# vsois/hanabi-agents

Hardware: AMD Instinct MI355X
Metric: env_steps_per_sec (higher is better)
Workload: dtype u8 env/encoder + bfloat16 Q-net GEMM (fp32 accumulate, fp32 master weights)

## Files before the change

### hanabi-agents_amd/csrc/actor_fused.hip

```cpp
#include <hip/hip_runtime.h>
#include <hip/hip_bf16.h>
#include <hip/hip_fp16.h>

#include <cstdint>
#include <type_traits>

#include "../../include/hanabi_hip.h"
#include "common.hpp"
#include "env_kernel.hpp"

using hb::fail;

namespace {

typedef __bf16 bf16x8 __attribute__((ext_vector_type(8)));
typedef _Float16 f16x8 __attribute__((ext_vector_type(8)));
typedef float f32x4 __attribute__((ext_vector_type(4)));

constexpr int FM = 128;
constexpr int FH = 512;
constexpr int FNT = 512;
constexpr int FK = 51;
constexpr int S2 = FH / 32;
constexpr int LUT_BYTES = 65536;
constexpr int H_BYTES = FM * FH * 2;
constexpr int FRAG_FLOATS = 3 * 8 * FM;
constexpr int LDS_TOTAL = H_BYTES + FRAG_FLOATS * 4;
constexpr float NEG_BIG = -1e30f;

struct FusedArgs {
  const uint32_t* obs;
  long long m;
  int words;
  int s1;
  const uint4* w1f;
  const float* b1;
  const uint4* w2f;
  const float* b2;
  const float* support;
  float* q;
  int n_actions, n_pass;
  const int8_t* legal;
  int32_t* actions;
  float epsilon;
  unsigned long long seed, draw;
  long long first_gid;
  unsigned long long* stamps;
};

#if defined(__HIP_DEVICE_COMPILE__)
typedef const __attribute__((address_space(4))) unsigned char KargByte;
typedef const __attribute__((address_space(4))) hb::EnvArgs KargEnv;
constexpr size_t ENV_KARG_OFF = (sizeof(FusedArgs) + alignof(hb::EnvArgs) - 1) / alignof(hb::EnvArgs) * alignof(hb::EnvArgs);
#define HB_ENV_KARGS(NAME)                                            \
  auto NAME##_kargs_ = __builtin_amdgcn_kernarg_segment_ptr();        \
  asm volatile("" : "+s"(NAME##_kargs_));                             \
  KargEnv& NAME = *(KargEnv*)((KargByte*)NAME##_kargs_ + ENV_KARG_OFF)
#else
#define HB_ENV_KARGS(NAME) const hb::EnvArgs NAME{}
#endif

#ifdef HB_STAMPS
#define HB_FSTAMP(slot)                                                                              \
  do {                                                                                               \
    __builtin_amdgcn_sched_barrier(0);                                                               \
    unsigned long long hb_t_;                                                                        \
    asm volatile("s_memtime %0\n\ts_waitcnt lgkmcnt(0)" : "=s"(hb_t_)::"memory");                    \
    if (a.stamps && lane == 0) a.stamps[(static_cast<long long>(blockIdx.x) * 8 + wave) * 16 + (slot)] = hb_t_; \
    __builtin_amdgcn_sched_barrier(0);                                                               \
  } while (0)
#define HB_FSTAMP_REAL(slot)                                                                         \
  do {                                                                                               \
    unsigned long long hb_t_;                                                                        \
    asm volatile("s_memrealtime %0\n\ts_waitcnt lgkmcnt(0)" : "=s"(hb_t_)::"memory");                \
    if (a.stamps && lane == 0) a.stamps[(static_cast<long long>(blockIdx.x) * 8 + wave) * 16 + (slot)] = hb_t_; \
  } while (0)
#else
#define HB_FSTAMP(slot) do {} while (0)
#define HB_FSTAMP_REAL(slot) do {} while (0)
#endif

template <bool F16>
__device__ __forceinline__ uint32_t pack16(float lo, float hi) {
  if constexpr (F16) {
    const _Float16 a = static_cast<_Float16>(lo), b = static_cast<_Float16>(hi);
    uint16_t ua, ub;
    __builtin_memcpy(&ua, &a, 2);
    __builtin_memcpy(&ub, &b, 2);
    return static_cast<uint32_t>(ua) | (static_cast<uint32_t>(ub) << 16);
  } else {
    const __hip_bfloat16 a = __float2bfloat16(lo), b = __float2bfloat16(hi);
    return static_cast<uint32_t>(*reinterpret_cast<const uint16_t*>(&a)) |
           (static_cast<uint32_t>(*reinterpret_cast<const uint16_t*>(&b)) << 16);
  }
}
template <bool F16>
__device__ __forceinline__ uint32_t bits2_one(uint32_t b, int p) {
  const uint32_t t = (b >> (2 * p)) & 3u;
  return __umul24((t | (t << 15)) & 0x00010001u, F16 ? 0x3C00u : 0x3F80u);
}
template <bool F16>
__device__ __forceinline__ f32x4 mfma16(const uint4& wv, const uint4& xv, const f32x4& c) {
  if constexpr (F16) {
    union { uint4 u; f16x8 f; } w, x;
    w.u = wv; x.u = xv;
    return __builtin_amdgcn_mfma_f32_16x16x32_f16(w.f, x.f, c, 0, 0, 0);
  } else {
    union { uint4 u; bf16x8 f; } w, x;
    w.u = wv; x.u = xv;
    return __builtin_amdgcn_mfma_f32_16x16x32_bf16(w.f, x.f, c, 0, 0, 0);
  }
}
typedef float f32x2 __attribute__((ext_vector_type(2)));
typedef unsigned int u32x2 __attribute__((ext_vector_type(2)));
__device__ __forceinline__ float vmax(float a, float b) {
  float r;
  asm("v_max_f32 %0, %1, %2" : "=v"(r) : "v"(a), "v"(b));
  return r;
}
__device__ __forceinline__ float vmax3(float a, float b, float c) {
  float r;
  asm("v_max3_f32 %0, %1, %2, %3" : "=v"(r) : "v"(a), "v"(b), "v"(c));
  return r;
}
__device__ __forceinline__ float exp2_fast(float x) { return __builtin_amdgcn_exp2f(x); }

template <bool F16, class K, int EG>
__device__ __forceinline__ void actor_fused_body(const FusedArgs& a) {
  __shared__ __attribute__((aligned(16))) unsigned char lds[LDS_TOTAL];
  const int tid = threadIdx.x, lane = tid & 63;
  const int wave = __builtin_amdgcn_readfirstlane(tid >> 6);
  const int r = lane & 15, qd = lane >> 4;
  const long long row0 = static_cast<long long>(blockIdx.x) * FM;
  const int s1 = a.s1, G = (s1 + 3) >> 2;
  unsigned char* lutb = lds + (LDS_TOTAL - LUT_BYTES);
  const int bits_off = LDS_TOTAL - LUT_BYTES - 2048 * G;
  unsigned char* bits = lds + bits_off;
  const int m_early = bits_off >> 14;

  HB_FSTAMP_REAL(14);
  HB_FSTAMP(0);
  const uint4* w1p = a.w1f + (4 * wave) * 64 + lane;
  uint4 wa[4], wb[4];
#pragma unroll
  for (int n = 0; n < 4; ++n) wa[n] = w1p[n * 64];

  uint32_t w[4] = {0u, 0u, 0u, 0u};
  auto load_item = [&](int it) {
    const int rr = it & (FM - 1), g = it >> 7;
    long long row = row0 + rr;
    if (row >= a.m) row = a.m - 1;
    const uint32_t* src = a.obs + row * a.words + 4 * g;
#pragma unroll
    for (int i = 0; i < 4; ++i) w[i] = (4 * g + i < a.words) ? src[i] : 0u;
  };
  if (tid < FM * G) load_item(tid);
  for (int e = tid; e < 4096; e += FNT) {
    const uint32_t v = static_cast<uint32_t>(e) >> 4;
    *reinterpret_cast<uint4*>(lutb + e * 16) = make_uint4(bits2_one<F16>(v, 0), bits2_one<F16>(v, 1), bits2_one<F16>(v, 2), bits2_one<F16>(v, 3));
  }
  for (int it = tid; it < FM * G; it += FNT) {
    const int rr = it & (FM - 1), g = it >> 7;
    if (it != tid) load_item(it);
    uint32_t* dst = reinterpret_cast<uint32_t*>(bits) + (static_cast<size_t>((rr >> 4) * G + g) * 64 + (rr & 15));
#pragma unroll
    for (int qq = 0; qq < 4; ++qq) {
      const uint32_t o = ((w[0] >> (8 * qq)) & 0xFFu) | (((w[1] >> (8 * qq)) & 0xFFu) << 8) | (((w[2] >> (8 * qq)) & 0xFFu) << 16) |
                         (((w[3] >> (8 * qq)) & 0xFFu) << 24);
      dst[qq * 16] = o;
    }
  }
  HB_FSTAMP(1);
  __syncthreads();
  HB_FSTAMP(2);

  f32x4 acc[4][8];
#pragma unroll
  for (int n = 0; n < 4; ++n) {
    const float4 b = *reinterpret_cast<const float4*>(a.b1 + 64 * wave + 16 * n + 4 * qd);
#pragma unroll
    for (int m = 0; m < 8; ++m) acc[n][m] = f32x4{b.x, b.y, b.z, b.w};
  }

  {
    const unsigned char* lut = lutb + r * 16;
    const uint32_t* bw = reinterpret_cast<const uint32_t*>(bits) + lane;
#define HB_L1_STEP(I, WCUR, WNXT, HAVE_NEXT)                                                                   \
  {                                                                                                            \
    const int s_ = 4 * g + (I);                                                                                \
    if (HAVE_NEXT) {                                                                                           \
      _Pragma("unroll") for (int n = 0; n < 4; ++n) WNXT[n] = w1p[(s_ + 1) * 2048 + n * 64];                    \
    }                                                                                                          \
// ... 44 lines not shown
  HB_FSTAMP(4);
  __syncthreads();
  HB_H_WRITE(m >= m_early)
#undef HB_H_WRITE

  HB_FSTAMP(5);
  __syncthreads();
  HB_FSTAMP(6);

  const int n_pass = a.n_pass, A = a.n_actions;
  const int full_cap = 8 * n_pass;
  constexpr float LOG2E = 1.44269504088896340736f;
  const unsigned char* hrow = lds + r * 1024;

  for (int p = 0; p < n_pass; ++p) {
    const int slot = 8 * p + wave;
    {
      const float* bp = a.b2 + static_cast<long long>(slot) * 64 + 4 * qd;
#pragma unroll
      for (int n = 0; n < 4; ++n) {
        const float4 b = *reinterpret_cast<const float4*>(bp + 16 * n);
#pragma unroll
        for (int m = 0; m < 8; ++m) acc[n][m] = f32x4{b.x, b.y, b.z, b.w};
      }
    }
    const uint4* wp = w2p + static_cast<long long>(p) * S2 * 2048;
#define HB_L2_HALF(S, WCUR, M0)                                                                                \
  {                                                                                                            \
    uint4 xf[4];                                                                                               \
    const int ch = ((4 * (S) + qd) ^ r) << 4;                                                                  \
    _Pragma("unroll") for (int m = 0; m < 4; ++m) xf[m] = *reinterpret_cast<const uint4*>(hrow + ((M0) + m) * 16384 + ch); \
    _Pragma("unroll") for (int n = 0; n < 4; ++n) {                                                            \
      _Pragma("unroll") for (int m = 0; m < 4; ++m)                                                            \
        acc[n][(M0) + m] = mfma16<F16>(WCUR[n], xf[m], acc[n][(M0) + m]);                                      \
    }                                                                                                          \
  }
#define HB_L2_STEP(S, WCUR, WNXT, HAVE_NEXT)                                                                   \
  {                                                                                                            \
    if (HAVE_NEXT) {                                                                                           \
      _Pragma("unroll") for (int n = 0; n < 4; ++n) WNXT[n] = wp[((S) + 1) * 2048 + n * 64];                    \
    }                                                                                                          \
    asm volatile("" ::: "memory");                                                                             \
    HB_L2_HALF(S, WCUR, 0)                                                                                     \
    __builtin_amdgcn_sched_barrier(0);                                                                         \
    HB_L2_HALF(S, WCUR, 4)                                                                                     \
  }
#pragma unroll 1
    for (int s = 0; s < S2; s += 2) {
      HB_L2_STEP(s, wa, wb, true)
      HB_L2_STEP(s + 1, wb, wa, (s + 2 < S2))
    }
#undef HB_L2_STEP
#undef HB_L2_HALF
    if (p < 2) HB_FSTAMP(7 + 3 * p);
    if (p + 1 < n_pass) {
#pragma unroll
      for (int n = 0; n < 4; ++n) wa[n] = wp[S2 * 2048 + n * 64];
    }

    auto sup_at = [&](int k) { return a.support[k < FK ? k : FK - 1]; };
    f32x2 supF[6];
#pragma unroll
    for (int i = 0; i < 6; ++i) supF[i] = f32x2{sup_at(4 * (2 * i) + qd), sup_at(4 * (2 * i + 1) + qd)};
    const float supF12 = sup_at(48 + qd);
    const int fq = wave & 3;
    const f32x2 supZa = f32x2{sup_at(13 * fq + qd), sup_at(13 * fq + 4 + qd)};
    const f32x2 supZb = f32x2{sup_at(13 * fq + 8 + qd), sup_at(13 * fq + 12)};
    const bool full_ok = slot < A && slot < full_cap;
    float* fb = reinterpret_cast<float*>(lds + H_BYTES) + wave * FM;
    const f32x2 L2 = f32x2{LOG2E, LOG2E};
    hb::static_for<2>([&](auto MH) {
    constexpr int M0 = 4 * decltype(MH)::value;
    float qF[4], zm[4], zs[4], zt[4], vf12[4], vz3[4], nmx[4], nmz[4];
#define HB_M for (int m = 0; m < 4; ++m)
#define HB_SWAP16(X, OP) { const u32x2 t_ = __builtin_amdgcn_permlane16_swap(__float_as_uint(X), __float_as_uint(X), false, false); \
                           X = OP(__uint_as_float(t_.x), __uint_as_float(t_.y)); }
#define HB_SWAP32(X, OP) { const u32x2 t_ = __builtin_amdgcn_permlane32_swap(__float_as_uint(X), __float_as_uint(X), false, false); \
                           X = OP(__uint_as_float(t_.x), __uint_as_float(t_.y)); }
#define HB_ADD(A_, B_) ((A_) + (B_))
#pragma unroll
    HB_M { vf12[m] = qd < 3 ? acc[3][M0 + m][0] : NEG_BIG; vz3[m] = qd == 3 ? acc[3][M0 + m][0] : NEG_BIG; }
#pragma unroll
    HB_M nmx[m] = vmax3(acc[0][M0 + m][0], acc[0][M0 + m][1], acc[0][M0 + m][2]);
#pragma unroll
    HB_M nmx[m] = vmax3(nmx[m], acc[0][M0 + m][3], acc[1][M0 + m][0]);
#pragma unroll
    HB_M nmx[m] = vmax3(nmx[m], acc[1][M0 + m][1], acc[1][M0 + m][2]);
#pragma unroll
    HB_M nmx[m] = vmax3(nmx[m], acc[1][M0 + m][3], acc[2][M0 + m][0]);
#pragma unroll
    HB_M nmx[m] = vmax3(nmx[m], acc[2][M0 + m][1], acc[2][M0 + m][2]);
#pragma unroll
    HB_M nmx[m] = vmax3(nmx[m], acc[2][M0 + m][3], vf12[m]);
#pragma unroll
    HB_M nmz[m] = vmax(vmax3(acc[3][M0 + m][1], acc[3][M0 + m][2], acc[3][M0 + m][3]), vz3[m]);
#pragma unroll
    HB_M HB_SWAP16(nmx[m], vmax)
#pragma unroll
    HB_M HB_SWAP16(nmz[m], vmax)
#pragma unroll
    HB_M HB_SWAP32(nmx[m], vmax)
#pragma unroll
    HB_M HB_SWAP32(nmz[m], vmax)
#pragma unroll
    HB_M { nmx[m] *= -LOG2E; nmz[m] *= -LOG2E; }
    f32x2 s2[4], t2[4];
#define HB_PAIR_FIRST(N, LO, SUP)                                                                   \
// ... 25 lines not shown
      sF[m] = s2[m].x + s2[m].y + e12;
      tF[m] = t2[m].x + t2[m].y + e12 * supF12;
    }
#pragma unroll
    HB_M {
      const f32x2 arg = f32x2{acc[3][M0 + m][1], acc[3][M0 + m][2]} * L2 + f32x2{nmz[m], nmz[m]};
      const f32x2 e = f32x2{exp2_fast(arg.x), exp2_fast(arg.y)};
      s2[m] = e;
      t2[m] = e * supZa;
    }
#pragma unroll
    HB_M {
      const f32x2 arg = f32x2{acc[3][M0 + m][3], vz3[m]} * L2 + f32x2{nmz[m], nmz[m]};
      const f32x2 e = f32x2{exp2_fast(arg.x), exp2_fast(arg.y)};
      s2[m] += e;
      t2[m] += e * supZb;
    }
#pragma unroll
    HB_M { zs[m] = s2[m].x + s2[m].y; zt[m] = t2[m].x + t2[m].y; }
#pragma unroll
    HB_M HB_SWAP16(sF[m], HB_ADD)
#pragma unroll
    HB_M HB_SWAP16(tF[m], HB_ADD)
#pragma unroll
    HB_M HB_SWAP16(zs[m], HB_ADD)
#pragma unroll
    HB_M HB_SWAP16(zt[m], HB_ADD)
#pragma unroll
    HB_M HB_SWAP32(sF[m], HB_ADD)
#pragma unroll
    HB_M HB_SWAP32(tF[m], HB_ADD)
#pragma unroll
    HB_M HB_SWAP32(zs[m], HB_ADD)
#pragma unroll
    HB_M HB_SWAP32(zt[m], HB_ADD)
#pragma unroll
    HB_M { zm[m] = -nmz[m]; qF[m] = tF[m] * __builtin_amdgcn_rcpf(sF[m]) * (1.0f / FK); }
#undef HB_M
#undef HB_SWAP16
#undef HB_SWAP32
#undef HB_ADD
    if (qd == 0) {
#pragma unroll
      for (int m = 0; m < 4; ++m) {
        const long long row = row0 + 16 * (M0 + m) + r;
        if (full_ok && row < a.m) a.q[row * A + slot] = qF[m];
        fb[16 * (M0 + m) + r] = zm[m];
        fb[8 * FM + 16 * (M0 + m) + r] = zs[m];
        fb[16 * FM + 16 * (M0 + m) + r] = zt[m];
      }
    }
    __builtin_amdgcn_sched_barrier(0);
    });
    if (p < 2) HB_FSTAMP(8 + 3 * p);
    __syncthreads();
    if (tid < 2 * FM) {
      const int rr = tid & (FM - 1), g = tid >> 7;
      const int ea = full_cap + 2 * p + g;
      const long long row = row0 + rr;
      if (ea < A && row < a.m) {
        const float* f = reinterpret_cast<const float*>(lds + H_BYTES) + (4 * g) * FM + rr;
        const float m0 = f[0], m1 = f[FM], m2 = f[2 * FM], m3 = f[3 * FM];
        const float M = fmaxf(fmaxf(m0, m1), fmaxf(m2, m3));
        const float e0 = exp2_fast(m0 - M), e1 = exp2_fast(m1 - M), e2 = exp2_fast(m2 - M), e3 = exp2_fast(m3 - M);
        const float* fs = f + 8 * FM;
        const float* ft = f + 16 * FM;
        const float S = fs[0] * e0 + fs[FM] * e1 + fs[2 * FM] * e2 + fs[3 * FM] * e3;
        const float T = ft[0] * e0 + ft[FM] * e1 + ft[2 * FM] * e2 + ft[3 * FM] * e3;
        a.q[row * A + ea] = T * __builtin_amdgcn_rcpf(S) * (1.0f / FK);
      }
    }
    if (p + 1 < n_pass) __syncthreads();
    if (p < 2) HB_FSTAMP(9 + 3 * p);
  }
  [[maybe_unused]] uint32_t rf_flag[2] = {0u, 0u}, rf_ep[2] = {0u, 0u};
  if constexpr (!std::is_void_v<K>) {
    if (wave >= 2) {
      HB_ENV_KARGS(env);
#pragma unroll
      for (int h = 0; h < 2; ++h) {
        const long long g = row0 + 64 * h + lane;
        if (g < env.n) {
          rf_flag[h] = env.refill[g];
          rf_ep[h] = env.state[g * K::SW + 6];
        }
      }
    }
  }
  if (a.legal) {
    asm volatile("s_waitcnt vmcnt(0)" ::: "memory");
    __syncthreads();
    if (tid < FM && row0 + tid < a.m) {
      const long long g = row0 + tid;
      const unsigned long long gid = static_cast<unsigned long long>(a.first_gid + g);
      uint32_t rnd[4];
      hb::philox4x32_10(static_cast<uint32_t>(a.draw), static_cast<uint32_t>(a.draw >> 32), static_cast<uint32_t>(gid),
                        static_cast<uint32_t>(gid >> 32), static_cast<uint32_t>(a.seed), static_cast<uint32_t>(a.seed >> 32), rnd);
      const float* qr = a.q + g * A;
      const int8_t* lr = a.legal + g * A;
      float best = -INFINITY;
      unsigned long long legal_mask = 0, ties = 0;
      for (int i = 0; i < A; ++i) {
        const float v = __hip_atomic_load(qr + i, __ATOMIC_RELAXED, __HIP_MEMORY_SCOPE_AGENT);
        if (lr[i] != 0) {
          legal_mask |= 1ull << i;
          if (v > best) { best = v; ties = 1ull << i; }
          else if (v == best) ties |= 1ull << i;
        }
      }
      const float u = static_cast<float>(rnd[0] >> 8) * (1.0f / 16777216.0f);
      unsigned long long pool = (u < a.epsilon) ? legal_mask : ties;
      if (pool == 0) pool = legal_mask;
      int pick = 0;
      const int c = __popcll(pool);
      if (c > 0) {
        int k = static_cast<int>(__umulhi(rnd[1], static_cast<uint32_t>(c)));
        while (k-- > 0) pool &= pool - 1;
        pick = __ffsll(static_cast<long long>(pool)) - 1;
      }
      a.actions[g] = pick;
      if constexpr (!std::is_void_v<K>) reinterpret_cast<int*>(lds + H_BYTES)[tid] = pick;
    }
  }
  if constexpr (!std::is_void_v<K>) {
    static_assert(K::LIFE >= 2, "a deck flagged by one launch is regenerated by the next: a game must outlive the step after its deal");
    if (wave >= 2) {
      HB_ENV_KARGS(env);
      int turn = wave - 2;
#pragma unroll
      for (int h = 0; h < 2; ++h) {
        unsigned long long todo = __ballot(rf_flag[h] != 0u);
        while (todo) {
          const int src = __ffsll(static_cast<long long>(todo)) - 1;
          todo &= todo - 1;
          if (turn == 0) {
            const long long g = row0 + 64 * h + src;
            hb::refill_deck<K>(env, g, lane, [&] {
              return static_cast<uint32_t>(__builtin_amdgcn_readlane(static_cast<int>(rf_ep[h]), src));
            });
            if (lane == 0) env.refill[g] = 0;
            turn = 6;
          }
          --turn;
        }
      }
      asm volatile("s_waitcnt vmcnt(0)" ::: "memory");
    }
    constexpr int ENV_WORDS = hb::env_lds_words<K, EG>();
    static_assert((FM / EG) * ENV_WORDS * 4 <= H_BYTES && FM / EG <= FNT / 64, "env tail: the LDS slices must fit in H");
    __syncthreads();
    if (wave < FM / EG) {
      HB_ENV_KARGS(env);
      const long long g0 = row0 + EG * wave;
      const int uid = lane < EG ? reinterpret_cast<const int*>(lds + H_BYTES)[EG * wave + lane] : 0;
      hb::env_wave_step<K, EG>(env, g0, lane, reinterpret_cast<uint32_t*>(lds) + wave * ENV_WORDS, uid, g0 / EG);
    }
  }
  HB_FSTAMP_REAL(15);
}

template <bool F16>
__global__ __launch_bounds__(FNT) void actor_fused_kernel(const FusedArgs a) {
  actor_fused_body<F16, void, 16>(a);
}

template <bool F16, class K, int EG>
__global__ __launch_bounds__(FNT) void actor_env_fused_kernel(const FusedArgs a, const hb::EnvArgs env) {
  (void)env;
  actor_fused_body<F16, K, EG>(a);
}

template <bool F16>
__global__ __launch_bounds__(FNT) void actor_fused_grouped_kernel(const FusedArgs a, const hb_fused_tile* __restrict__ tiles) {
  const hb_fused_tile& t = tiles[blockIdx.x];
  if (!t.active) return;
  FusedArgs b = a;
  b.w1f = static_cast<const uint4*>(t.w1f); b.b1 = t.b1f; b.w2f = static_cast<const uint4*>(t.w2f); b.b2 = t.b2f;
  b.support = t.support;
  b.first_gid = t.first_game_id - static_cast<long long>(blockIdx.x) * FM;
  actor_fused_body<F16, void, 16>(b);
}

struct PackArgs {
  const __hip_bfloat16* w1; int w1_ld;
  const __hip_bfloat16* b1;
  const __hip_bfloat16* w2; int w2_ld;
  const __hip_bfloat16* b2;
  int obs_len, s1, n_actions, n_pass;
  uint4* w1f; float* b1f; uint4* w2f; float* b2f;
  int chunks1, chunks2;
  int f16;
  uint16_t* w1t; int w1t_ld;
  uint16_t* w2t; int w2t_ld;
};
__device__ __forceinline__ float bias_to_float(const __hip_bfloat16* b, int i, int f16) {
  return f16 ? __half2float(reinterpret_cast<const __half*>(b)[i]) : __bfloat162float(b[i]);
}
__host__ __device__ __forceinline__ int fused_logit(int col, int n_actions, int n_pass) {
  const int slot = col >> 6, c = col & 63, n = c >> 4, q = (c >> 2) & 3, j = c & 3;
  const int r16 = 4 * n + j;
  const int full_cap = 8 * n_pass;
  int action, atom;
  if (r16 < 12 || (r16 == 12 && q < 3)) {
    action = slot < full_cap ? slot : n_actions;
    if (action >= n_actions) return -1;
    atom = r16 < 12 ? 4 * r16 + q : 48 + q;
  } else {
    const int p = slot >> 3, w = slot & 7, f = w & 3;
    action = full_cap + 2 * p + (w >> 2);
    atom = r16 == 12 ? 13 * f + 12 : 13 * f + 4 * (r16 - 13) + q;
// ... 197 lines not shown
    a.first_gid = sel->first_gid;
  }
  *launch = true;
  return HB_OK;
}

static int fused_launch(const uint32_t* obs_bits_dev, int64_t n_rows, int32_t obs_len, const void* w1f_dev, const float* b1f_dev,
                        const void* w2f_dev, const float* b2f_dev, const float* support_dev, int32_t hidden, int32_t n_actions,
                        int32_t n_atoms, float* q_dev, unsigned long long* stamps_dev, const FusedSelect* sel, int32_t dtype, void* stream) {
  FusedArgs a;
  bool go = false;
  if (int rc = fused_args(obs_bits_dev, n_rows, obs_len, w1f_dev, b1f_dev, w2f_dev, b2f_dev, support_dev, hidden, n_actions, n_atoms, q_dev,
                          stamps_dev, sel, dtype, a, &go))
    return rc;
  if (!go) return HB_OK;
  const dim3 grid(static_cast<unsigned>((n_rows + FM - 1) / FM));
  if (dtype == 2) hipLaunchKernelGGL(actor_fused_kernel<true>, grid, dim3(FNT), 0, static_cast<hipStream_t>(stream), a);
  else hipLaunchKernelGGL(actor_fused_kernel<false>, grid, dim3(FNT), 0, static_cast<hipStream_t>(stream), a);
  HB_HIP(hipGetLastError());
  return HB_OK;
}

}

namespace {

using ActEnvFull2 = hb::Cfg<2, 5, 5, 5, 8, 3>;
using ActEnvFull5 = hb::Cfg<5, 5, 5, 4, 8, 3>;
constexpr int ENV_EG = 16;

template <class K>
static bool is_cfg(const hb::EnvVariant& v) {
  return v.P == K::P && v.C == K::C && v.R == K::R && v.H == K::H && v.INFO == K::INFO && v.LIFE == K::LIFE;
}

template <bool F16, class K>
static void launch_act_env(const FusedArgs& a, const hb::EnvArgs& env, dim3 grid, hipStream_t stream) {
  if (env.ev_start && env.ev_stop)
    hipExtLaunchKernelGGL((actor_env_fused_kernel<F16, K, ENV_EG>), grid, dim3(FNT), 0, stream, env.ev_start, env.ev_stop, 0, a, env);
  else
    hipLaunchKernelGGL((actor_env_fused_kernel<F16, K, ENV_EG>), grid, dim3(FNT), 0, stream, a, env);
}

}

namespace hb {

bool actor_env_fused_supported(const EnvVariant& v) { return is_cfg<ActEnvFull2>(v) || is_cfg<ActEnvFull5>(v); }

int actor_env_fused_launch(const uint32_t* obs_bits_dev, const int8_t* legal_dev, int64_t n_rows, int32_t obs_len, const void* w1f_dev,
                           const float* b1f_dev, const void* w2f_dev, const float* b2f_dev, const float* support_dev, int32_t hidden,
                           int32_t n_actions, int32_t n_atoms, float* q_dev, float epsilon, uint64_t seed, uint64_t draw,
                           int64_t first_game_id, int32_t* actions_dev, int32_t dtype, const EnvArgs& env, const EnvVariant& var,
                           void* stream) {
  if (!legal_dev || !actions_dev) return fail(HB_ERR_INVALID, "null argument");
  if (!actor_env_fused_supported(var)) return fail(HB_ERR_INVALID, "no fused policy + env kernel for this game configuration");
  if (n_rows != env.n) return fail(HB_ERR_INVALID, "n_rows (%lld) must equal the env's game count (%lld)", static_cast<long long>(n_rows), env.n);
  if (n_actions != var.n_actions || obs_len != var.obs_len) return fail(HB_ERR_INVALID, "actor shape does not match the env");
  const FusedSelect sel{legal_dev, actions_dev, epsilon, seed, draw, first_game_id};
  FusedArgs a;
  bool go = false;
  if (int rc = fused_args(obs_bits_dev, n_rows, obs_len, w1f_dev, b1f_dev, w2f_dev, b2f_dev, support_dev, hidden, n_actions, n_atoms, q_dev,
                          nullptr, &sel, dtype, a, &go))
    return rc;
  if (!go) return HB_OK;
  const dim3 grid(static_cast<unsigned>((n_rows + FM - 1) / FM));
  const hipStream_t st = static_cast<hipStream_t>(stream);
  const bool f16 = dtype == 2;
  if (is_cfg<ActEnvFull2>(var)) {
    if (f16) launch_act_env<true, ActEnvFull2>(a, env, grid, st);
    else launch_act_env<false, ActEnvFull2>(a, env, grid, st);
  } else {
    if (f16) launch_act_env<true, ActEnvFull5>(a, env, grid, st);
    else launch_act_env<false, ActEnvFull5>(a, env, grid, st);
  }
  HB_HIP(hipGetLastError());
  return HB_OK;
}

}
```

### hanabi-agents_amd/csrc/env_api.hip

```cpp
#include <hip/hip_runtime.h>

#include <cstdarg>
#include <cstdio>
#include <cstdlib>
#include <cstring>
#include <new>
#include <string>
#include <vector>

#include "../../include/hanabi_hip.h"
#include "common.hpp"
#include "env_kernel.hpp"

namespace hb {
const EnvVariant* variants_full(int* n);
const EnvVariant* variants_small(int* n);
const EnvVariant* variants_vsmall(int* n);

thread_local std::string g_error;
int fail(int code, const char* fmt, ...) {
  char buf[512];
  va_list ap;
  va_start(ap, fmt);
  vsnprintf(buf, sizeof buf, fmt, ap);
// ... 435 lines not shown
                       float* reward_dev, int8_t* terminal_dev, float* agent_reward_dev, int8_t* agent_step_type_dev,
                       int8_t* score_dev, void* stream) {
  if (!e) return fail(HB_ERR_INVALID, "null env");
  if (!actions_dev) return fail(HB_ERR_INVALID, "actions_dev is required");
  if (int rc = check_out_packed(obs_bits_dev, obs_dev, legal_dev)) return rc;
  hb::EnvArgs a{};
  a.mode = hb::MODE_STEP;
  a.actions = actions_dev;
  a.obs = obs_dev;
  a.obs_bits = obs_bits_dev;
  a.legal = legal_dev;
  a.reward = reward_dev;
  a.terminal = terminal_dev;
  a.agent_reward = agent_reward_dev;
  a.agent_step_type = agent_step_type_dev;
  a.score = score_dev;
  if (int rc = join_refill(e, stream)) return rc;
  if (int rc = launch(e, a, stream)) return rc;
  return refill_async(e, stream);
}

int hb_env_step_select_packed(hb_env* e, const float* q_dev, const int8_t* sel_legal_dev, float epsilon, uint64_t seed, uint64_t draw,
                              int64_t first_game_id, int32_t* actions_out_dev, uint32_t* obs_bits_dev, int8_t* obs_dev,
                              int8_t* legal_dev, float* reward_dev, int8_t* terminal_dev, float* agent_reward_dev,
                              int8_t* agent_step_type_dev, int8_t* score_dev, void* stream) {
  if (!e) return fail(HB_ERR_INVALID, "null env");
  if (!q_dev || !sel_legal_dev || !actions_out_dev) return fail(HB_ERR_INVALID, "q_dev, sel_legal_dev and actions_out_dev are required");
  if ((reinterpret_cast<uintptr_t>(q_dev) & 15) || (reinterpret_cast<uintptr_t>(sel_legal_dev) & 3))
    return fail(HB_ERR_ALIGN, "q_dev must be 16-byte and sel_legal_dev 4-byte aligned");
  if (e->var->n_actions > 64) return fail(HB_ERR_INVALID, "the fused selection handles at most 64 actions");
  if (int rc = check_out_packed(obs_bits_dev, obs_dev, legal_dev)) return rc;
  hb::EnvArgs a{};
  a.mode = hb::MODE_STEP;
  a.sel_q = q_dev;
  a.sel_legal = sel_legal_dev;
  a.sel_actions = actions_out_dev;
  a.sel_eps = epsilon;
  a.sel_seed = seed;
  a.sel_draw = draw;
  a.sel_first_gid = first_game_id;
  a.obs = obs_dev;
  a.obs_bits = obs_bits_dev;
  a.legal = legal_dev;
  a.reward = reward_dev;
  a.terminal = terminal_dev;
  a.agent_reward = agent_reward_dev;
  a.agent_step_type = agent_step_type_dev;
  a.score = score_dev;
  if (int rc = join_refill(e, stream)) return rc;
  if (int rc = launch(e, a, stream)) return rc;
  return refill_async(e, stream);
}

int hb_actor_fused_act_step(hb_env* e, const uint32_t* obs_bits_dev, const int8_t* legal_dev, int64_t n_rows, int32_t obs_len,
                            const void* w1f_dev, const float* b1f_dev, const void* w2f_dev, const float* b2f_dev, const float* support_dev,
                            int32_t hidden, int32_t n_actions, int32_t n_atoms, float* q_dev, float epsilon, uint64_t seed, uint64_t draw,
                            int64_t first_game_id, int32_t* actions_dev, int32_t dtype, uint32_t* obs_bits_out_dev, int8_t* legal_out_dev,
                            float* reward_dev, int8_t* terminal_dev, float* agent_reward_dev, int8_t* agent_step_type_dev,
                            int8_t* score_dev, void* stream) {
  if (!e) return fail(HB_ERR_INVALID, "null env");
  if (e->shuffled) return fail(HB_ERR_INVALID, "the fused policy + env kernel has no colour-permuted form: step a shuffled env with "
                                               "hb_env_step_packed or hb_env_step_select_packed");
  if (int rc = check_out_packed(obs_bits_out_dev, nullptr, legal_out_dev)) return rc;
  hb::EnvArgs a{};
  a.mode = hb::MODE_STEP;
  a.obs_bits = obs_bits_out_dev;
  a.legal = legal_out_dev;
  a.reward = reward_dev;
  a.terminal = terminal_dev;
  a.agent_reward = agent_reward_dev;
  a.agent_step_type = agent_step_type_dev;
  a.score = score_dev;
  prepare(e, a);
  if (int rc = join_refill(e, stream)) return rc;
  if (int rc = hb::actor_env_fused_launch(obs_bits_dev, legal_dev, n_rows, obs_len, w1f_dev, b1f_dev, w2f_dev, b2f_dev, support_dev, hidden,
                                          n_actions, n_atoms, q_dev, epsilon, seed, draw, first_game_id, actions_dev, dtype, a, *e->var,
                                          stream))
    return rc;
  e->since_refill = 1;
  return HB_OK;
}

int hb_actor_fused_step_supported(const hb_env* e) { return e && !e->shuffled && hb::actor_env_fused_supported(*e->var) ? 1 : 0; }

#ifdef HB_STAMPS
int hb_env_step_stamped(hb_env* e, const int32_t* actions_dev, int8_t* obs_dev, int8_t* legal_dev,
                        unsigned long long* stamps_dev, void* stream) {
  hb::EnvArgs a{};
  a.mode = hb::MODE_STEP;
  a.actions = actions_dev;
  a.obs = obs_dev;
  a.legal = legal_dev;
  a.stamps = stamps_dev;
  if (int rc = join_refill(e, stream)) return rc;
  if (int rc = launch(e, a, stream)) return rc;
  return refill_async(e, stream);
}
#endif

int hb_env_illegal_count(hb_env* e, int64_t* out) {
  if (!e || !out) return fail(HB_ERR_INVALID, "null argument");
  unsigned long long v = 0;
  HB_HIP(hipMemcpy(&v, e->illegal, 8, hipMemcpyDeviceToHost));
  *out = static_cast<int64_t>(v);
  return HB_OK;
}

int hb_env_stats(hb_env* e, int64_t* episodes, int64_t* score_sum) {
  if (!e || !episodes || !score_sum) return fail(HB_ERR_INVALID, "null argument");
  std::vector<unsigned long long> v(static_cast<size_t>(2 * e->stat_slots));
  HB_HIP(hipMemcpy(v.data(), e->illegal + 1, 16 * e->stat_slots, hipMemcpyDeviceToHost));
  unsigned long long ep = 0, sc = 0;
  for (long long i = 0; i < e->stat_slots; ++i) { ep += v[2 * i]; sc += v[2 * i + 1]; }
  *episodes = static_cast<int64_t>(ep);
  *score_sum = static_cast<int64_t>(sc);
  return HB_OK;
}

int hb_env_set_refill_period(hb_env* e, int32_t steps) {
  if (!e) return fail(HB_ERR_INVALID, "null env");
  if (steps < 1 || steps > e->cfg.max_life) return fail(HB_ERR_INVALID, "refill period must be 1..max_life (%d)", e->cfg.max_life);
  e->refill_period = steps;
  return HB_OK;
}

int hb_env_set_async_refill(hb_env* e, int32_t on) {
  if (!e) return fail(HB_ERR_INVALID, "null env");
  HB_HIP(hipDeviceSynchronize());
  e->refill_in_flight = false;
  e->async_refill = on != 0;
  return HB_OK;
}

int hb_env_export_state(hb_env* e, uint32_t* rows_dev, void* stream) {
  if (!e || !rows_dev) return fail(HB_ERR_INVALID, "null argument");
  HB_HIP(hipMemcpyAsync(rows_dev, e->state, static_cast<size_t>(e->n) * e->var->state_words * 4, hipMemcpyDeviceToDevice,
                        static_cast<hipStream_t>(stream)));
  return HB_OK;
}
const uint32_t* hb_env_state(hb_env* e) { return e ? e->state : nullptr; }

int hb_env_import_state(hb_env* e, const uint32_t* rows_dev, void* stream) {
  if (!e || !rows_dev) return fail(HB_ERR_INVALID, "null argument");
  HB_HIP(hipMemcpyAsync(e->state, rows_dev, static_cast<size_t>(e->n) * e->var->state_words * 4, hipMemcpyDeviceToDevice,
                        static_cast<hipStream_t>(stream)));
  if (int rc = join_refill(e, stream)) return rc;
  HB_HIP(hipMemsetAsync(e->refill, 1, static_cast<size_t>(e->n), static_cast<hipStream_t>(stream)));
  if (int rc = draw_color_perms(e, stream)) return rc;
  return refill(e, stream);
// ... 61 lines not shown
```

### hanabi-agents_amd/csrc/env_kernel.hpp

```cpp
#pragma once
#include <hip/hip_runtime.h>
#include <hip/hip_ext.h>
#include <stdint.h>
#include <utility>

struct hb_config;

namespace hb {

enum { MODE_STEP = 0, MODE_OBSERVE = 1, MODE_RESET = 2 };
constexpr int NEXT_DECK_BYTES = 64;
enum { MV_PLAY = 0, MV_DISCARD = 1, MV_RCOLOR = 2, MV_RRANK = 3 };

struct EnvArgs {
  uint32_t* state;
  const int32_t* actions;
  const uint8_t* mask;
  const uint8_t* decks;
  uint8_t* next_deck;
  uint8_t* refill;
  int8_t* obs;
  uint32_t* obs_bits;
  int8_t* legal;
  float* reward;
// ... 909 lines not shown
    for (int i = 0; i < K::NW; ++i) ob[i] = acc.w[i];
#pragma unroll
    for (int i = K::NW; i < K::NWP; ++i) ob[i] = 0;
    uint32_t* lb = lbits + lane * K::LW;
    lb[0] = static_cast<uint32_t>(legal);
    lb[1] = static_cast<uint32_t>(legal >> 32);
    lb[2] = 0;
  }
  wave_sync();
  if (a.obs_bits) {
    uint32_t* dst = a.obs_bits + g0 * K::NW;
    for (int e = lane; e < nvalid * K::NW; e += 64) {
      const int g = e / K::NW, i = e - g * K::NW;
      dst[e] = obits[g * K::NWP + i];
    }
  }
  if (a.obs) expand_rows<K::OBS_LEN>(obits, K::NWP, nvalid, a.obs + g0 * K::OBS_LEN, lane);
  if (a.legal) expand_rows<K::A>(lbits, K::LW, nvalid, a.legal + g0 * K::A, lane);
}

template <class K, int G>
void launch_encode(const EncodeArgs& a, hipStream_t stream) {
  const long long per_block = 4LL * G;
  const unsigned blocks = static_cast<unsigned>((a.n + per_block - 1) / per_block);
  if (blocks == 0) return;
  hipLaunchKernelGGL((encode_rows_kernel<K, G>), dim3(blocks), dim3(256), 0, stream, a);
}

using LaunchFn = void (*)(const EnvArgs&, hipStream_t);
using EncodeFn = void (*)(const EncodeArgs&, hipStream_t);
struct EnvVariant {
  int P, C, R, H, INFO, LIFE;
  int obs_len, n_actions, deck, state_words;
  LaunchFn g8, g16, g32, g64, refill;
  LaunchFn s8, s16, s32, s64;
  EncodeFn e16, e32;
};

template <class K>
constexpr EnvVariant make_variant() {
  return EnvVariant{K::P, K::C, K::R, K::H, K::INFO, K::LIFE, K::OBS_LEN, K::A, K::D, K::SW,
                    &launch_env<K, 8>, &launch_env<K, 16>, &launch_env<K, 32>, &launch_env<K, 64>, &launch_refill<K>,
                    &launch_env_shuf<K, 8>, &launch_env_shuf<K, 16>, &launch_env_shuf<K, 32>, &launch_env_shuf<K, 64>,
                    &launch_encode<K, 16>, &launch_encode<K, 32>};
}

const EnvVariant* find_variant(const ::hb_config* c);

bool actor_env_fused_supported(const EnvVariant& v);
int actor_env_fused_launch(const uint32_t* obs_bits_dev, const int8_t* legal_dev, int64_t n_rows, int32_t obs_len, const void* w1f_dev,
                           const float* b1f_dev, const void* w2f_dev, const float* b2f_dev, const float* support_dev, int32_t hidden,
                           int32_t n_actions, int32_t n_atoms, float* q_dev, float epsilon, uint64_t seed, uint64_t draw,
                           int64_t first_game_id, int32_t* actions_dev, int32_t dtype, const EnvArgs& env, const EnvVariant& var,
                           void* stream);

}
```

Baseline: 321.1 million.

## Vectorize action-selection loads with buffer loads and overlap Philox before barrier

The epsilon-greedy selection tail now builds the legal-action mask from wide buffer loads issued before the block barrier, and computes the Philox random draw while those loads are in flight. The Q-value scan uses 128-bit buffer loads with a cache-policy bit instead of per-element relaxed atomic loads, with template dispatch on action count and alignment. Stamp plumbing for the fused kernel is also added but is compiled out unless HB_STAMPS is defined. The aim is to cut serialized scalar global loads in the per-row selection loop, in exchange for more register use and code-size growth from the templated variants.

```diff
diff --git a/hanabi-agents_amd/csrc/actor_fused.hip b/hanabi-agents_amd/csrc/actor_fused.hip
--- a/hanabi-agents_amd/csrc/actor_fused.hip
+++ b/hanabi-agents_amd/csrc/actor_fused.hip
@@ -75,10 +75,30 @@
     asm volatile("s_memrealtime %0\n\ts_waitcnt lgkmcnt(0)" : "=s"(hb_t_)::"memory");                \
     if (a.stamps && lane == 0) a.stamps[(static_cast<long long>(blockIdx.x) * 8 + wave) * 16 + (slot)] = hb_t_; \
   } while (0)
+#define HB_FSTAMP_HOLD(i)                                                                            \
+  do {                                                                                               \
+    __builtin_amdgcn_sched_barrier(0);                                                               \
+    asm volatile("s_memtime %0\n\ts_waitcnt lgkmcnt(0)" : "=s"(hb_hold_[i])::"memory");              \
+    __builtin_amdgcn_sched_barrier(0);                                                               \
+  } while (0)
+#define HB_FSTAMP_FLUSH()                                                                            \
+  do {                                                                                               \
+    if (a.stamps && a.legal && lane == 0) {                                                          \
+      for (int i_ = 0; i_ < 4; ++i_) a.stamps[(static_cast<long long>(blockIdx.x) * 8 + wave) * 16 + 9 + i_] = hb_hold_[i_]; \
+    }                                                                                                \
+  } while (0)
 #else
 #define HB_FSTAMP(slot) do {} while (0)
 #define HB_FSTAMP_REAL(slot) do {} while (0)
+#define HB_FSTAMP_HOLD(i) do {} while (0)
+#define HB_FSTAMP_FLUSH() do {} while (0)
 #endif
+#define HB_PSTAMP(k)                                                          \
+  do {                                                                        \
+    if (a.legal) { if (p == n_pass - 1 && (k) == 2) HB_FSTAMP_HOLD(0); }      \
+    else if (p == 0) HB_FSTAMP(7 + (k));                                      \
+    else if (p == 1) HB_FSTAMP(10 + (k));                                     \
+  } while (0)
 
 template <bool F16>
 __device__ __forceinline__ uint32_t pack16(float lo, float hi) {
@@ -125,6 +145,78 @@
 }
 __device__ __forceinline__ float exp2_fast(float x) { return __builtin_amdgcn_exp2f(x); }
 
+typedef unsigned int u32x4 __attribute__((ext_vector_type(4)));
+constexpr int SEL_RSRC_FLAGS = 0x00020000;
+constexpr int SEL_SC1 = 16;
+
+struct SelPick {
+  bool wide;
+  int nunit, ngrp;
+  __device__ __forceinline__ SelPick(int A, const void* q, const void* legal)
+      : wide((A & 3) == 0 && (reinterpret_cast<uintptr_t>(q) & 15) == 0 && (reinterpret_cast<uintptr_t>(legal) & 3) == 0),
+        nunit(wide ? A >> 2 : A), ngrp(wide ? (nunit + 3) >> 2 : (nunit + 15) >> 4) {}
+  template <class F>
+  __device__ __forceinline__ void operator()(F&& f) const {
+    hb::static_for<4>([&](auto G) {
+      constexpr int g = decltype(G)::value + 1;
+      if (ngrp == g) {
+        if (wide) f(std::true_type{}, std::integral_constant<int, 4 * g>{});
+        else f(std::false_type{}, std::integral_constant<int, 16 * g>{});
+      }
+    });
+  }
+};
+
+template <bool WIDE, int NU, class F>
+__device__ __forceinline__ unsigned long long sel_legal_mask(__amdgpu_buffer_rsrc_t rs, int off, int nunit, int A, F&& between) {
+  uint32_t w[NU];
+#pragma unroll
+  for (int u = 0; u < NU; ++u) {
+    const int uu = u < nunit ? u : nunit - 1;
+    if constexpr (WIDE) w[u] = __builtin_amdgcn_raw_buffer_load_b32(rs, off, 4 * uu, 0);
+    else w[u] = __builtin_amdgcn_raw_buffer_load_b8(rs, off, uu, 0);
+  }
+  __builtin_amdgcn_sched_barrier(0);
+  between();
+  unsigned long long m = 0;
+#pragma unroll
+  for (int u = 0; u < NU; ++u) {
+    if constexpr (WIDE) {
+#pragma unroll
+      for (int e = 0; e < 4; ++e) m |= static_cast<unsigned long long>(((w[u] >> (8 * e)) & 0xFFu) != 0u) << (4 * u + e);
+    } else {
+      m |= static_cast<unsigned long long>(w[u] != 0u) << u;
+    }
+  }
+  return A >= 64 ? m : m & ((1ull << A) - 1ull);
+}
+
+template <bool WIDE, int NU>
+__device__ __forceinline__ void sel_scan(__amdgpu_buffer_rsrc_t rs, int off, int nunit, unsigned long long legal_mask, float& best,
+                                         unsigned long long& ties) {
+  constexpr int E = WIDE ? 4 : 1;
+  float v[NU * E];
+#pragma unroll
+  for (int u = 0; u < NU; ++u) {
+    const int uu = u < nunit ? u : nunit - 1;
+    if constexpr (WIDE) {
+      const u32x4 x = __builtin_amdgcn_raw_buffer_load_b128(rs, off, 16 * uu, SEL_SC1);
+      v[4 * u] = __uint_as_float(x.x); v[4 * u + 1] = __uint_as_float(x.y);
+      v[4 * u + 2] = __uint_as_float(x.z); v[4 * u + 3] = __uint_as_float(x.w);
+    } else {
+      v[u] = __uint_as_float(__builtin_amdgcn_raw_buffer_load_b32(rs, off, 4 * uu, SEL_SC1));
+    }
+  }
+  __builtin_amdgcn_sched_barrier(0);
+#pragma unroll
+  for (int i = 0; i < NU * E; ++i) {
+    const bool lg = ((legal_mask >> i) & 1ull) != 0ull;
+    const bool gt = lg & (v[i] > best), eq = lg & (v[i] == best);
+    ties = gt ? 1ull << i : (eq ? ties | (1ull << i) : ties);
+    best = gt ? v[i] : best;
+  }
+}
+
 template <bool F16, class K, int EG>
 __device__ __forceinline__ void actor_fused_body(const FusedArgs& a) {
   __shared__ __attribute__((aligned(16))) unsigned char lds[LDS_TOTAL];
@@ -138,6 +230,9 @@
   unsigned char* bits = lds + bits_off;
   const int m_early = bits_off >> 14;
 
+#ifdef HB_STAMPS
+  unsigned long long hb_hold_[4] = {0ull, 0ull, 0ull, 0ull};
+#endif
   HB_FSTAMP_REAL(14);
   HB_FSTAMP(0);
   const uint4* w1p = a.w1f + (4 * wave) * 64 + lane;
@@ -288,7 +383,7 @@
     }
 #undef HB_L2_STEP
 #undef HB_L2_HALF
-    if (p < 2) HB_FSTAMP(7 + 3 * p);
+    HB_PSTAMP(0);
     if (p + 1 < n_pass) {
 #pragma unroll
       for (int n = 0; n < 4; ++n) wa[n] = wp[S2 * 2048 + n * 64];
@@ -420,7 +515,7 @@
     }
     __builtin_amdgcn_sched_barrier(0);
     });
-    if (p < 2) HB_FSTAMP(8 + 3 * p);
+    HB_PSTAMP(1);
     __syncthreads();
     if (tid < 2 * FM) {
       const int rr = tid & (FM - 1), g = tid >> 7;
@@ -439,7 +534,7 @@
       }
     }
     if (p + 1 < n_pass) __syncthreads();
-    if (p < 2) HB_FSTAMP(9 + 3 * p);
+    HB_PSTAMP(2);
   }
   [[maybe_unused]] uint32_t rf_flag[2] = {0u, 0u}, rf_ep[2] = {0u, 0u};
   if constexpr (!std::is_void_v<K>) {
@@ -456,26 +551,35 @@
     }
   }
   if (a.legal) {
+    const SelPick sel_pick(A, a.q, a.legal);
+    const bool sel_lane = tid < FM && row0 + tid < a.m;
+    const long long left = a.m - row0;
+    const int sel_bytes = static_cast<int>(left < FM ? left : FM) * A;
+    const int sel_off = tid * A;
+    uint32_t rnd[4] = {0u, 0u, 0u, 0u};
+    unsigned long long legal_mask = 0;
+    if (sel_lane) {
+      const __amdgpu_buffer_rsrc_t rs = __builtin_amdgcn_make_buffer_rsrc(const_cast<int8_t*>(a.legal) + row0 * A, 0, sel_bytes, SEL_RSRC_FLAGS);
+      sel_pick([&](auto W, auto N) {
+        legal_mask = sel_legal_mask<decltype(W)::value, decltype(N)::value>(rs, sel_off, sel_pick.nunit, A, [&] {
+          const unsigned long long gid = static_cast<unsigned long long>(a.first_gid + row0 + tid);
+          hb::philox4x32_10(static_cast<uint32_t>(a.draw), static_cast<uint32_t>(a.draw >> 32), static_cast<uint32_t>(gid),
+                            static_cast<uint32_t>(gid >> 32), static_cast<uint32_t>(a.seed), static_cast<uint32_t>(a.seed >> 32), rnd);
+        });
+      });
+    }
     asm volatile("s_waitcnt vmcnt(0)" ::: "memory");
+    HB_FSTAMP_HOLD(1);
     __syncthreads();
-    if (tid < FM && row0 + tid < a.m) {
+    HB_FSTAMP_HOLD(2);
+    if (sel_lane) {
       const long long g = row0 + tid;
-      const unsigned long long gid = static_cast<unsigned long long>(a.first_gid + g);
-      uint32_t rnd[4];
-      hb::philox4x32_10(static_cast<uint32_t>(a.draw), static_cast<uint32_t>(a.draw >> 32), static_cast<uint32_t>(gid),
-                        static_cast<uint32_t>(gid >> 32), static_cast<uint32_t>(a.seed), static_cast<uint32_t>(a.seed >> 32), rnd);
-      const float* qr = a.q + g * A;
-      const int8_t* lr = a.legal + g * A;
+      const __amdgpu_buffer_rsrc_t rs = __builtin_amdgcn_make_buffer_rsrc(a.q + row0 * A, 0, 4 * sel_bytes, SEL_RSRC_FLAGS);
       float best = -INFINITY;
-      unsigned long long legal_mask = 0, ties = 0;
-      for (int i = 0; i < A; ++i) {
-        const float v = __hip_atomic_load(qr + i, __ATOMIC_RELAXED, __HIP_MEMORY_SCOPE_AGENT);
-        if (lr[i] != 0) {
-          legal_mask |= 1ull << i;
-          if (v > best) { best = v; ties = 1ull << i; }
-          else if (v == best) ties |= 1ull << i;
-        }
-      }
+      unsigned long long ties = 0;
+      sel_pick([&](auto W, auto N) {
+        sel_scan<decltype(W)::value, decltype(N)::value>(rs, 4 * sel_off, sel_pick.nunit, legal_mask, best, ties);
+      });
       const float u = static_cast<float>(rnd[0] >> 8) * (1.0f / 16777216.0f);
       unsigned long long pool = (u < a.epsilon) ? legal_mask : ties;
       if (pool == 0) pool = legal_mask;
@@ -516,7 +620,10 @@
     }
     constexpr int ENV_WORDS = hb::env_lds_words<K, EG>();
     static_assert((FM / EG) * ENV_WORDS * 4 <= H_BYTES && FM / EG <= FNT / 64, "env tail: the LDS slices must fit in H");
+    HB_FSTAMP_HOLD(3);
     __syncthreads();
+    HB_FSTAMP(13);
+    HB_FSTAMP_FLUSH();
     if (wave < FM / EG) {
       HB_ENV_KARGS(env);
       const long long g0 = row0 + EG * wave;
@@ -524,6 +631,7 @@
       hb::env_wave_step<K, EG>(env, g0, lane, reinterpret_cast<uint32_t*>(lds) + wave * ENV_WORDS, uid, g0 / EG);
     }
   }
+  if constexpr (std::is_void_v<K>) HB_FSTAMP_FLUSH();
   HB_FSTAMP_REAL(15);
 }
 
@@ -827,7 +935,7 @@
                            const float* b1f_dev, const void* w2f_dev, const float* b2f_dev, const float* support_dev, int32_t hidden,
                            int32_t n_actions, int32_t n_atoms, float* q_dev, float epsilon, uint64_t seed, uint64_t draw,
                            int64_t first_game_id, int32_t* actions_dev, int32_t dtype, const EnvArgs& env, const EnvVariant& var,
-                           void* stream) {
+                           void* stream, unsigned long long* stamps_dev) {
   if (!legal_dev || !actions_dev) return fail(HB_ERR_INVALID, "null argument");
   if (!actor_env_fused_supported(var)) return fail(HB_ERR_INVALID, "no fused policy + env kernel for this game configuration");
   if (n_rows != env.n) return fail(HB_ERR_INVALID, "n_rows (%lld) must equal the env's game count (%lld)", static_cast<long long>(n_rows), env.n);
@@ -836,7 +944,7 @@
   FusedArgs a;
   bool go = false;
   if (int rc = fused_args(obs_bits_dev, n_rows, obs_len, w1f_dev, b1f_dev, w2f_dev, b2f_dev, support_dev, hidden, n_actions, n_atoms, q_dev,
-                          nullptr, &sel, dtype, a, &go))
+                          stamps_dev, &sel, dtype, a, &go))
     return rc;
   if (!go) return HB_OK;
   const dim3 grid(static_cast<unsigned>((n_rows + FM - 1) / FM));
diff --git a/hanabi-agents_amd/csrc/env_api.hip b/hanabi-agents_amd/csrc/env_api.hip
--- a/hanabi-agents_amd/csrc/env_api.hip
+++ b/hanabi-agents_amd/csrc/env_api.hip
@@ -511,12 +511,12 @@
   return refill_async(e, stream);
 }
 
-int hb_actor_fused_act_step(hb_env* e, const uint32_t* obs_bits_dev, const int8_t* legal_dev, int64_t n_rows, int32_t obs_len,
-                            const void* w1f_dev, const float* b1f_dev, const void* w2f_dev, const float* b2f_dev, const float* support_dev,
-                            int32_t hidden, int32_t n_actions, int32_t n_atoms, float* q_dev, float epsilon, uint64_t seed, uint64_t draw,
-                            int64_t first_game_id, int32_t* actions_dev, int32_t dtype, uint32_t* obs_bits_out_dev, int8_t* legal_out_dev,
-                            float* reward_dev, int8_t* terminal_dev, float* agent_reward_dev, int8_t* agent_step_type_dev,
-                            int8_t* score_dev, void* stream) {
+static int fused_act_step(hb_env* e, const uint32_t* obs_bits_dev, const int8_t* legal_dev, int64_t n_rows, int32_t obs_len,
+                          const void* w1f_dev, const float* b1f_dev, const void* w2f_dev, const float* b2f_dev, const float* support_dev,
+                          int32_t hidden, int32_t n_actions, int32_t n_atoms, float* q_dev, float epsilon, uint64_t seed, uint64_t draw,
+                          int64_t first_game_id, int32_t* actions_dev, int32_t dtype, uint32_t* obs_bits_out_dev, int8_t* legal_out_dev,
+                          float* reward_dev, int8_t* terminal_dev, float* agent_reward_dev, int8_t* agent_step_type_dev,
+                          int8_t* score_dev, unsigned long long* fused_stamps_dev, unsigned long long* env_stamps_dev, void* stream) {
   if (!e) return fail(HB_ERR_INVALID, "null env");
   if (e->shuffled) return fail(HB_ERR_INVALID, "the fused policy + env kernel has no colour-permuted form: step a shuffled env with "
                                                "hb_env_step_packed or hb_env_step_select_packed");
@@ -530,14 +530,26 @@
   a.agent_reward = agent_reward_dev;
   a.agent_step_type = agent_step_type_dev;
   a.score = score_dev;
+  a.stamps = env_stamps_dev;
   prepare(e, a);
   if (int rc = join_refill(e, stream)) return rc;
   if (int rc = hb::actor_env_fused_launch(obs_bits_dev, legal_dev, n_rows, obs_len, w1f_dev, b1f_dev, w2f_dev, b2f_dev, support_dev, hidden,
                                           n_actions, n_atoms, q_dev, epsilon, seed, draw, first_game_id, actions_dev, dtype, a, *e->var,
-                                          stream))
+                                          stream, fused_stamps_dev))
     return rc;
   e->since_refill = 1;
   return HB_OK;
+}
+
+int hb_actor_fused_act_step(hb_env* e, const uint32_t* obs_bits_dev, const int8_t* legal_dev, int64_t n_rows, int32_t obs_len,
+                            const void* w1f_dev, const float* b1f_dev, const void* w2f_dev, const float* b2f_dev, const float* support_dev,
+                            int32_t hidden, int32_t n_actions, int32_t n_atoms, float* q_dev, float epsilon, uint64_t seed, uint64_t draw,
+                            int64_t first_game_id, int32_t* actions_dev, int32_t dtype, uint32_t* obs_bits_out_dev, int8_t* legal_out_dev,
+                            float* reward_dev, int8_t* terminal_dev, float* agent_reward_dev, int8_t* agent_step_type_dev,
+                            int8_t* score_dev, void* stream) {
+  return fused_act_step(e, obs_bits_dev, legal_dev, n_rows, obs_len, w1f_dev, b1f_dev, w2f_dev, b2f_dev, support_dev, hidden, n_actions, n_atoms,
+                        q_dev, epsilon, seed, draw, first_game_id, actions_dev, dtype, obs_bits_out_dev, legal_out_dev, reward_dev, terminal_dev,
+                        agent_reward_dev, agent_step_type_dev, score_dev, nullptr, nullptr, stream);
 }
 
 int hb_actor_fused_step_supported(const hb_env* e) { return e && !e->shuffled && hb::actor_env_fused_supported(*e->var) ? 1 : 0; }
@@ -554,6 +566,17 @@
   if (int rc = join_refill(e, stream)) return rc;
   if (int rc = launch(e, a, stream)) return rc;
   return refill_async(e, stream);
+}
+int hb_actor_fused_act_step_stamped(hb_env* e, const uint32_t* obs_bits_dev, const int8_t* legal_dev, int64_t n_rows, int32_t obs_len,
+                            const void* w1f_dev, const float* b1f_dev, const void* w2f_dev, const float* b2f_dev, const float* support_dev,
+                            int32_t hidden, int32_t n_actions, int32_t n_atoms, float* q_dev, float epsilon, uint64_t seed, uint64_t draw,
+                            int64_t first_game_id, int32_t* actions_dev, int32_t dtype, uint32_t* obs_bits_out_dev, int8_t* legal_out_dev,
+                            float* reward_dev, int8_t* terminal_dev, float* agent_reward_dev, int8_t* agent_step_type_dev,
+                            int8_t* score_dev, unsigned long long* fused_stamps_dev, unsigned long long* env_stamps_dev,
+                                    void* stream) {
+  return fused_act_step(e, obs_bits_dev, legal_dev, n_rows, obs_len, w1f_dev, b1f_dev, w2f_dev, b2f_dev, support_dev, hidden, n_actions, n_atoms,
+                        q_dev, epsilon, seed, draw, first_game_id, actions_dev, dtype, obs_bits_out_dev, legal_out_dev, reward_dev, terminal_dev,
+                        agent_reward_dev, agent_step_type_dev, score_dev, fused_stamps_dev, env_stamps_dev, stream);
 }
 #endif
 
diff --git a/hanabi-agents_amd/csrc/env_kernel.hpp b/hanabi-agents_amd/csrc/env_kernel.hpp
--- a/hanabi-agents_amd/csrc/env_kernel.hpp
+++ b/hanabi-agents_amd/csrc/env_kernel.hpp
@@ -985,6 +985,6 @@
                            const float* b1f_dev, const void* w2f_dev, const float* b2f_dev, const float* support_dev, int32_t hidden,
                            int32_t n_actions, int32_t n_atoms, float* q_dev, float epsilon, uint64_t seed, uint64_t draw,
                            int64_t first_game_id, int32_t* actions_dev, int32_t dtype, const EnvArgs& env, const EnvVariant& var,
-                           void* stream);
-
-}
+                           void* stream, unsigned long long* stamps_dev = nullptr);
+
+}
```

Result: no change. 322.9 million (median of 6 runs) (+0.6%).
